# MoonLab-YH/AOD_MEH_HUA

Measured on AMD Instinct MI355X. Metric: images/sec train+HUA-score, RetinaNet-R50 VOC 512^2, higher is better.
Workload: dtype bf16x3

## Files before the change

aod_meh_hua_amd/_C.py:

```python
import ctypes as C
import os

import torch

_HERE = os.path.dirname(os.path.abspath(__file__))
LIB_PATH = os.environ.get('AOD_HIP_LIB') or os.path.join(_HERE, 'lib', 'libaodhip.so')


class AodHipError(RuntimeError):
    pass


if not os.path.exists(LIB_PATH):
    raise ImportError(f'{LIB_PATH} is missing: run `python -m aod_meh_hua_amd.build` (hipcc, gfx950). '
                      'There is no CPU fallback for the MEH/HUA hot path.')
lib = C.CDLL(LIB_PATH)


class ConvSeg(C.Structure):
    _fields_ = [('B', C.c_int32), ('H', C.c_int32), ('W', C.c_int32), ('OH', C.c_int32), ('OW', C.c_int32),
                ('src_row0', C.c_int64), ('dst_row0', C.c_int64)]


class ConvDesc(C.Structure):
    _fields_ = [('C', C.c_int32), ('N', C.c_int32), ('R', C.c_int32), ('S', C.c_int32), ('stride', C.c_int32),
                ('pad', C.c_int32), ('dil', C.c_int32), ('transposed', C.c_int32), ('relu', C.c_int32),
                ('out_f32', C.c_int32), ('nseg', C.c_int32), ('x3', C.c_int32), ('seg', ConvSeg * 8)]


P, I32, I64, F32, U64, SZ = C.c_void_p, C.c_int32, C.c_int64, C.c_float, C.c_uint64, C.c_size_t
_SIGS = {
    'aod_version': (C.c_int, []),
    'aod_conv_x3p_count': (C.c_int64, []),
    'aod_set_pointwise_mode': (C.c_int, [I32]),
    'aod_bottleneck64_fwd': (C.c_int, [P, I32, I32, I32, I32, P, P, P, P, P, P, P, P, P, P, P, P]),
    'aod_bottleneck64x3_fwd': (C.c_int, [P, I32, I32, I32, I32, P, P, P, P, P, P, P, P, P, P, P, P]),
    'aod_bottleneck64x3_ds_fwd': (C.c_int, [P, I32, I32, I32, P, P, P, P, P, P, P, P, P, P, P, P, P, P]),
    'aod_bottleneck64_ds_fwd': (C.c_int, [P, I32, I32, I32, P, P, P, P, P, P, P, P, P, P, P, P, P, P]),
    'aod_halo_conv3x3_x3_applies': (C.c_int, [P]),
    'aod_halo_conv3x3_x3': (C.c_int, [P, P, P, P, P, P]),
    'aod_mfma_clock_probe': (C.c_int, [I32, I32, P, P, P]),
    'aod_bottleneck128x3_bwd': (C.c_int, [P, I32, I32, I32, P, P, P, P, P, P, P, P, P, P, P, P, P]),
    'aod_bottleneck128x3_fwd': (C.c_int, [P, I32, I32, I32, P, P, P, P, P, P, P, P, P, P, P, P, P]),
    'aod_bottleneck128_fwd': (C.c_int, [P, I32, I32, I32, P, P, P, P, P, P, P, P, P, P, P, P, P]),
    'aod_frag_pack': (C.c_int, [P, I32, I32, P]),
    'aod_frag_pack_item_bytes': (C.c_int, []),
    'aod_bottleneck256f_fwd': (C.c_int, [P, I32, I32, I32, P, P, P, P, P, P, P, P, P, P, P, P, P]),
    'aod_bottleneck256f_bwd': (C.c_int, [P, I32, I32, I32, P, P, P, P, P, P, P, P, P, P, P, P, P]),
    'aod_bottleneck_bwd': (C.c_int, [I32, P, I32, I32, I32, P, P, P, P, P, P, P, P, P, P, P, P, P]),
    'aod_bottleneck256_fwd': (C.c_int, [P, I32, I32, I32, P, P, P, P, P, P, P, P, P, P, P, P, P]),
    'aod_conv2d': (C.c_int, [C.POINTER(ConvDesc), P, P, P, P, P, P, P, P, P, P, P]),
    'aod_conv2d_ws_bytes': (SZ, [C.POINTER(ConvDesc)]),
    'aod_conv2d_ws': (C.c_int, [C.POINTER(ConvDesc), P, P, P, P, P, P, P, P, P, P, P, SZ, P]),
    'aod_conv2d_grouped': (C.c_int, [C.POINTER(ConvDesc), I32, P, P, P, P, P, P, P]),
    'aod_halo_conv3x3_applies': (C.c_int, [C.POINTER(ConvDesc)]),
    'aod_halo_conv3x3': (C.c_int, [C.POINTER(ConvDesc), P, P, P, P, P, P, P]),
    'aod_conv2d_wgrad': (C.c_int, [C.POINTER(ConvDesc), P, P, P, P, P]),
    'aod_conv2d_wgrad_splits': (C.c_int, [C.POINTER(ConvDesc)]),
    'aod_conv2d_wgrad_slabs': (C.c_int, [C.POINTER(ConvDesc), P, P, P, I32, I64, P, P]),
    'aod_conv2d_wgrad_group_plan': (C.c_int, [P, I32, P]),
    'aod_conv2d_wgrad_grouped': (C.c_int, [P, I32, P, P, P, P, P, P, P]),
    'aod_unpack_wgrad_slabs_grouped': (C.c_int, [I32, P, P, P, P, P, P, P, P, P, P, P, P, P, P, P, P, P]),
    'aod_unpack_wgrad_slabs': (C.c_int, [P, I32, I64, P, I32, I32, I32, I32, I32, I32, P, P, P, P, P, P, P]),
    'aod_conv_row_table_bytes': (SZ, [C.POINTER(ConvDesc)]),
    'aod_conv_row_table': (C.c_int, [C.POINTER(ConvDesc), P, P]),
    'aod_pack_weight_fwd': (C.c_int, [P, P, I32, I32, I32, I32, I32, P]),
    'aod_param_prep': (C.c_int, [P, I32, I32, P]),
    'aod_param_prep_item_bytes': (C.c_int, []),
    'aod_pack_weight_dgrad': (C.c_int, [P, P, I32, I32, I32, I32, I32, P, P]),
    'aod_unpack_wgrad': (C.c_int, [P, P, I32, I32, I32, I32, I32, I32, I32, P, P, P, P, P, P, P]),
    'aod_nchw_f32_to_nhwc_bf16': (C.c_int, [P, P, I32, I32, I32, I32, I32, P]),
    'aod_nchw_f32_to_s2d_bf16': (C.c_int, [P, P, I32, I32, I32, I32, P]),
    'aod_stem_pool_fwd': (C.c_int, [P, P, P, P, P, I32, I32, I32, P]),
    'aod_set_deterministic': (C.c_int, [I32]),
    'aod_get_deterministic': (C.c_int, []),
    'aod_stem_pool_x3_fwd': (C.c_int, [P, P, P, P, P, I32, I32, I32, I32, P]),
    'aod_maxpool3x3s2': (C.c_int, [P, P, I32, I32, I32, I32, P]),
    'aod_upsample2x_add': (C.c_int, [P, P, I32, I32, I32, I32, I32, I32, P]),
    'aod_upsample2x_add_bwd': (C.c_int, [P, P, I32, I32, I32, I32, I32, I32, P]),
    'aod_upsample2x_add_to': (C.c_int, [P, P, P, I32, I32, I32, I32, I32, I32, P]),
    'aod_upsample2x_add_bwd_set': (C.c_int, [P, P, I32, I32, I32, I32, I32, I32, P]),
    'aod_act_bwd': (C.c_int, [P, P, P, P, P, P, P, P, P, P, I64, I32, I32, I32, P]),
    'aod_add_relu': (C.c_int, [P, P, P, I64, P]),
    'aod_pad_cast_colsum': (C.c_int, [P, P, P, P, I64, I32, I32, I32, P]),
    'aod_assign_ws_bytes': (SZ, [I32, I32]),
    'aod_max_iou_assign': (C.c_int, [P, P, I64, I32, P, P, P, I32, F32, F32, F32, I32, I32, P, P, P, P, P, P, P, P, P, I32, P, P]),
    'aod_loss_partials_len': (SZ, [I64]),
    'aod_edl_focal_l1_fwd': (C.c_int, [P, P, P, P, P, P, I64, I32, F32, F32, P, P, P, P]),
    'aod_edl_focal_l1_bwd': (C.c_int, [P, P, P, P, P, P, I64, I32, F32, F32, P, P, P, F32, I32, P, P, I32, I32, I32, I32, P]),
    'aod_edl_focal_elem': (C.c_int, [P, P, I64, I32, F32, F32, P, P, P]),
    'aod_meh_loss_fwd': (C.c_int, [P, P, P, I64, P, P, P]),
    'aod_meh_loss_bwd': (C.c_int, [P, P, P, I64, P, P, I32, I32, I32, P]),
    'aod_loss_levels_partials_len': (SZ, [I32, P]),
    'aod_edl_focal_l1_levels_fwd': (C.c_int, [P, P, P, P, P, P, I32, P, I32, F32, F32, P, P, P, P, I32, P, P, P]),
    'aod_edl_focal_l1_levels_bwd': (C.c_int, [P, P, P, P, P, P, I32, P, I32, F32, F32, P, P, P, P, P, I32, I32, I32, I32, P]),
    'aod_meh_loss_levels_fwd': (C.c_int, [P, P, P, I32, P, P, P, P]),
    'aod_meh_loss_levels_bwd': (C.c_int, [P, P, P, I32, P, P, P, I32, I32, I32, P]),
    'aod_softmax_rowmax': (C.c_int, [P, I32, I64, I32, F32, P, P, I32, P]),
    'aod_topk_stable': (C.c_int, [P, I32, I64, I32, P, I64, P]),
    'aod_pre_nms_levels': (C.c_int, [I32, P, P, P, P, P, P, I32, I32, F32, I32, I32, P, P, P, P, F32, P, P, P, P, P, P, P, I64, P]),
    'aod_gather_decode': (C.c_int, [P, P, P, P, P, I32, I64, I32, I32, I64, P, P, P, P, F32, P, P, P, P, I64, I64, I64, I32, P]),
    'aod_nms_ws_bytes': (SZ, [I32, I32, I32]),
    'aod_multiclass_nms': (C.c_int, [P, P, I32, I32, I32, F32, F32, I32, P, P, P, P, P, P]),
    'aod_hua_ws_bytes': (SZ, [I32, I32]),
    'aod_hua_score': (C.c_int, [P, P, P, P, P, P, P, P, P, I32, I32, I32, I32, I32, F32, F32, F32, I32, U64, P, I32, I32, I32, P, P, I32, P, P, P]),
    'aod_maxpool_fwd': (C.c_int, [P, P, I32, I32, I32, I32, I32, I32, I32, I32, I32, P]),
    'aod_maxpool_bwd': (C.c_int, [P, P, P, I32, I32, I32, I32, I32, I32, I32, I32, I32, P]),
    'aod_l2norm_fwd': (C.c_int, [P, P, P, I64, I32, F32, P]),
    'aod_l2norm_bwd': (C.c_int, [P, P, P, P, P, I64, I32, F32, P]),
    'aod_ssd_loss_fwd': (C.c_int, [P, P, P, P, P, P, I32, I32, I32, I32, I32, F32, P, P, P, P]),
    'aod_ssd_loss_bwd': (C.c_int, [P, P, P, P, P, P, P, P, I32, I32, I32, I32, F32, P, P, P, P, P, P]),
    'aod_synth_normal_images': (C.c_int, [P, I32, I64, U64, P, P]),
    'aod_image_xform': (C.c_int, [P, P, I32, I32, I32, P, P]),
    'aod_x3_split': (C.c_int, [P, P, I64, I32, P]),
    'aod_x3_merge': (C.c_int, [P, P, I64, I32, P]),
    'aod_x3_add': (C.c_int, [P, P, P, I64, P]),
    'aod_x3_nchw_f32_to_s2d': (C.c_int, [P, P, I32, I32, I32, I32, P]),
    'aod_x3_maxpool3x3s2': (C.c_int, [P, P, I32, I32, I32, I32, P]),
    'aod_x3_upsample2x_add_to': (C.c_int, [P, P, P, I32, I32, I32, I32, I32, I32, P]),
    'aod_x3_upsample2x_add_bwd_set': (C.c_int, [P, P, I32, I32, I32, I32, I32, I32, P]),
    'aod_x3_act_bwd': (C.c_int, [P, P, P, P, I64, I32, I32, P]),
    'aod_x3_pad_cast_colsum': (C.c_int, [P, P, P, P, I64, I32, P]),
    'aod_x3_nchw_f32_to_nhwc': (C.c_int, [P, P, I32, I32, I32, I32, P]),
    'aod_x3_maxpool_fwd': (C.c_int, [P, P, I32, I32, I32, I32, I32, I32, I32, I32, I32, P]),
    'aod_x3_maxpool_bwd': (C.c_int, [P, P, P, I32, I32, I32, I32, I32, I32, I32, I32, I32, P]),
    'aod_x3_l2norm_fwd': (C.c_int, [P, P, P, I64, I32, F32, P]),
    'aod_x3_l2norm_bwd': (C.c_int, [P, P, P, P, P, I64, I32, F32, P]),
    'aod_sgd_multi': (C.c_int, [P, P, P, P, I32, F32, P, F32, F32, I32, F32, P]),
}
for _n, (_r, _a) in _SIGS.items():
    if hasattr(lib, _n):
        getattr(lib, _n).restype = _r
        getattr(lib, _n).argtypes = _a
lib.aod_last_error.restype = C.c_char_p


def ptr(t):
    if t is None:
        return None
    if not t.is_cuda:
        raise AodHipError('aod_meh_hua_amd ops need tensors on the MI355X (cuda:N); got a CPU tensor. There is no CPU fallback.')
    return C.c_void_p(t.data_ptr())


def stream():
    return C.c_void_p(torch.cuda.current_stream().cuda_stream)


def check(rc, name='aod'):
    if rc != 0:
        raise AodHipError(f'{name} failed ({rc}): {lib.aod_last_error().decode()}')


def call(name, *args):
    check(getattr(lib, name)(*args), name)
```

aod_meh_hua_amd/csrc/conv.hip:

```cpp
#include "common.h"
#include "pointwise.h"
#include "conv_x3p.h"

struct ConvGroup { const bf16_t* x; const bf16_t* w; void* y; const float* pre_shift; const bf16_t* mask; float* colsum; };
struct ConvKParams {
  const bf16_t* x;
  const bf16_t* w;
  void* y;
  const float* pre_scale;
  const float* pre_shift;
  const bf16_t* res;
  const bf16_t* mask;
  const float* post_scale;
  bf16_t* zraw;
  float* colsum;
  int C, N, K, R, S, stride, pad, dil, transposed, relu, out_f32;
  int nseg, M;
  int tiles_m, tiles_n;
  int ksplit;
  float* ws;
  int perm;
  int ngroups;
  ConvGroup grp[4];
  int stagger;
// ... 879 lines not shown
    for (int j = 0; j < 8; ++j) sr[er][ec * 8 + j] = csum[j];
    __syncthreads();
    const int c = blockIdx.y * 256 + t;
    if (c < p.N) {
      float s2 = 0.f;
#pragma unroll
      for (int r = 0; r < 8; ++r) s2 += sr[r][t];
      if (p.cs_ws) p.cs_ws[(long long)blockIdx.x * p.N + c] = s2;
      else atomicAdd(p.colsum + c, s2);
    }
  }
}

static void x3p_args(const ConvKParams& p, X3PArgs& a) {
  memset(&a, 0, sizeof(a));
  a.x = p.x; a.w = p.w; a.y = reinterpret_cast<bf16_t*>(p.y); a.pre_scale = p.pre_scale; a.pre_shift = p.pre_shift; a.res = p.res; a.mask = p.mask;
  a.colsum = p.colsum; a.C = p.C; a.N = p.N; a.K = p.K; a.taps = p.R * p.S; a.S = p.S; a.stride = p.stride; a.pad = p.pad; a.dil = p.dil;
  a.transposed = p.transposed; a.relu = p.relu; a.nseg = p.nseg; a.M = p.M; a.x_bytes = p.x_bytes; a.w_bytes = p.w_bytes;
  a.tapin = (p.tap_inner && a.taps > 1 && p.C >= 256) ? 1 : 0;
  for (int i = 0; i < 8; ++i) {
    a.segH[i] = p.segH[i]; a.segW[i] = p.segW[i]; a.segOH[i] = p.segOH[i]; a.segOW[i] = p.segOW[i]; a.segB[i] = p.segB[i];
    a.seg_src0[i] = p.seg_src0[i]; a.seg_dst0[i] = p.seg_dst0[i]; a.seg_mend[i] = p.seg_mend[i];
  }
  if (p.ngroups > 1) {
    a.ngroups = p.ngroups;
    for (int g = 0; g < p.ngroups; ++g) {
      a.grp[g].x = p.grp[g].x; a.grp[g].w = p.grp[g].w; a.grp[g].y = reinterpret_cast<bf16_t*>(p.grp[g].y); a.grp[g].shift = p.grp[g].pre_shift;
      a.grp[g].mask = p.grp[g].mask; a.grp[g].colsum = p.grp[g].colsum;
    }
  }
}

static int choose_ksplit(const ConvKParams& p) {
  const int nk = (p.K + 63) / 64;
  if (nk < 64) return 1;
  static const char* dbg_hw = getenv("AOD_KSPLIT_MAXHW");
  const long long maxhw = dbg_hw ? atoll(dbg_hw) : 256;
  long long rows16 = 0;
  for (int i = 0; i < p.nseg; ++i) {
    if (p.segB[i] <= 0) continue;
    if ((long long)p.segOH[i] * p.segOW[i] > maxhw) return 1;
    rows16 += 16ll * p.segOH[i] * p.segOW[i];
  }
  static const char* dbg_ks = getenv("AOD_KSPLIT_STEPS");
  if (dbg_ks) { const int per = atoi(dbg_ks); return nk / per > 1 ? nk / per : 1; }
  const long long tiles = ((rows16 + 127) / 128) * ((p.N + 127) / 128);
  long long ks = 512 / (tiles > 0 ? tiles : 1);
  if (ks > nk / 8) ks = nk / 8;
  return ks > 1 ? (int)ks : 1;
}

static int conv_params(const aod_conv_desc_t* desc, const void* src, const void* w_packed, void* dst, const float* pre_scale,
                       const float* pre_shift, const void* res, const void* mask, const float* post_scale, void* zraw, float* colsum,
                       ConvKParams& p) {
  AOD_CHECK_ARG(desc && src && w_packed && dst, "conv: null pointer");
  memset(&p, 0, sizeof(p));
  int rc = fill_params(desc, p);
  if (rc) return rc;
  AOD_CHECK_ARG(!(desc->out_f32 && zraw), "conv: zraw needs a bf16 destination");
  if (desc->x3) {
    AOD_CHECK_ARG(!zraw && !post_scale, "conv (x3): zraw / post_scale are not supported");
    AOD_CHECK_ARG(desc->out_f32 || desc->N % 32 == 0, "conv (x3): a bf16 (X-layout) destination needs N %% 32 == 0, got %d", desc->N);
    AOD_CHECK_ARG(!(desc->out_f32 && (res || mask)), "conv (x3): residual / mask operands need an X-layout destination");
  }
  p.x = (const bf16_t*)src; p.w = (const bf16_t*)w_packed; p.y = dst;
  p.pre_scale = pre_scale; p.pre_shift = pre_shift; p.res = (const bf16_t*)res; p.mask = (const bf16_t*)mask;
  p.post_scale = post_scale; p.zraw = (bf16_t*)zraw; p.colsum = colsum;
  p.ksplit = 1;
  { static const char* dbg_st = getenv("AOD_STAGGER"); p.stagger = (dbg_st && dbg_st[0] == '0') ? 0 : 1; }
  { static const char* dbg_ti = getenv("AOD_X3_TAPS_INNER"); p.tap_inner = (dbg_ti && dbg_ti[0] == '0') ? 0 : 1; }
  p.perm = (desc->transposed && desc->stride == 2 && desc->R * desc->S > 1 && desc->R * desc->S <= 64) ? 1 : 0;
  if (desc->transposed && desc->stride == 2 && desc->R == 1 && desc->S == 1 && desc->pad == 0 && desc->nseg == 1 && res && res == dst &&
      !mask && !colsum && !pre_scale && !pre_shift && !post_scale && !zraw && !desc->relu && !desc->out_f32 && p.M > 0) {
    static const char* dbg_lat = getenv("AOD_DGRAD_LATTICE");
    if (!(dbg_lat && dbg_lat[0] == '0')) {
      p.up_w = p.segOW[0]; p.up_hw = p.segOH[0] * p.segOW[0];
      p.segOH[0] = p.segH[0]; p.segOW[0] = p.segW[0];
      p.stride = 1;
      const long long m = (long long)p.segB[0] * p.segH[0] * p.segW[0];
      p.M = (int)m;
      for (int i = 0; i < 8; ++i) p.seg_mend[i] = (int)m;
      p.bigrows = m >= (1ll << 22) ? 1 : 0;
    }
  }
  static const char* dbg_perm = getenv("AOD_DGRAD_CLASSES");
  if (dbg_perm && dbg_perm[0] == '0') p.perm = 0;
  long long xrows = 0;
  for (int i = 0; i < desc->nseg; ++i) {
    const aod_conv_seg_t& sg = desc->seg[i];
    AOD_CHECK_ARG(sg.src_row0 >= 0, "conv: negative src_row0");
    const long long e = sg.src_row0 + (long long)sg.B * sg.H * sg.W;
    if (e > xrows) xrows = e;
  }
  p.x_bytes = xrows * p.C * 2;
  p.w_bytes = (long long)p.N * p.K * 2;
  AOD_CHECK_ARG(p.x_bytes < 0xe0000000ll && p.w_bytes < 0xe0000000ll, "conv: operand larger than 3.5 GiB (32-bit buffer offsets)");
  return 0;
}

extern "C" size_t aod_conv2d_ws_bytes(const aod_conv_desc_t* desc) {
  ConvKParams p;
  memset(&p, 0, sizeof(p));
  if (!desc || fill_params(desc, p) != 0 || p.M == 0) return 0;
  const int ks = choose_ksplit(p);
  return ks > 1 ? (size_t)ks * p.M * p.N * 4 : 0;
}

extern "C" int aod_conv2d_ws(const aod_conv_desc_t* desc, const void* src, const void* w_packed, void* dst,
                             const float* pre_scale, const float* pre_shift, const void* res, const void* mask,
                             const float* post_scale, void* zraw, float* colsum, void* workspace, size_t workspace_bytes,
                             aod_stream_t stream) {
  ConvKParams p;
  int rc = conv_params(desc, src, w_packed, dst, pre_scale, pre_shift, res, mask, post_scale, zraw, colsum, p);
  if (rc) return rc;
  if (p.M == 0) return 0;
  hipStream_t st = (hipStream_t)stream;
  if (!p.x3 && !p.up_w && p.R == 1 && p.S == 1 && p.stride == 1 && p.pad == 0 && p.nseg == 1 && !p.out_f32 && !p.zraw && !p.post_scale) {
    PwArgs a;
    const long long s0 = p.seg_src0[0], d0 = p.seg_dst0[0];
    a.x = p.x + s0 * p.C; a.w = p.w; a.y = reinterpret_cast<bf16_t*>(p.y) + d0 * p.N;
    a.pre_scale = p.pre_scale; a.pre_shift = p.pre_shift;
    a.res = p.res ? p.res + d0 * p.N : nullptr; a.mask = p.mask ? p.mask + d0 * p.N : nullptr; a.colsum = p.colsum;
    a.M = p.M; a.N = p.N; a.K = p.C; a.relu = p.relu;
    if (aod_pw_wants(a)) return aod_pw_gemm(a, st);
  }
  const int ks = (workspace && !p.perm && !p.up_w) ? choose_ksplit(p) : 1;
  if (ks > 1) {
    const size_t need = (size_t)ks * p.M * p.N * 4;
    AOD_CHECK_ARG(workspace_bytes >= need, "conv: split-K workspace of %zu bytes, need %zu (aod_conv2d_ws_bytes)", workspace_bytes, need);
    p.ksplit = ks; p.ws = (float*)workspace;
    if (p.x3) { if (p.N > 64) launch_conv<128, 128, 256, 2, false, 2, true>(p, st); else launch_conv<128, 64, 256, 2, false, 2, true>(p, st); }
    else if (p.N > 64) launch_conv<128, 128>(p, st); else launch_conv<128, 64>(p, st);
    AOD_LAUNCH_CHECK();
    p.cs_ws = p.colsum ? aod_det_scratch((size_t)((p.M + 7) / 8) * p.N) : nullptr;
    hipLaunchKernelGGL(conv_splitk_finalize_kernel, dim3((p.M + 7) / 8, (p.N + 255) / 256), dim3(256), 0, st, p);
    AOD_LAUNCH_CHECK();
    if (p.cs_ws) return aod_colsum_finalize(p.cs_ws, (p.M + 7) / 8, p.N, p.N, p.colsum, nullptr, 0, st);
    return 0;
  }
  auto ntiles = [&](int bm, int bn) { return (long long)((p.M + bm - 1) / bm) * ((p.N + bn - 1) / bn); };
  static const char* dbg_want = getenv("AOD_TILE_WANT");
  const long long want = dbg_want ? atoll(dbg_want) : 512;
  const int pad128 = (p.N + 127) / 128 * 128, pad64 = (p.N + 63) / 64 * 64;
  const bool ragged = p.N > 128 && (pad128 - pad64) * 5 >= pad128;
  if (p.x3 && !p.out_f32 && !p.zraw && !p.post_scale && !p.bigrows && p.R == p.S) {
    const long long t256 = ntiles(256, 256);
    const bool big = !p.res && p.N % 256 == 0 && p.K >= 2048 && t256 >= 240 && t256 * 100 >= ((t256 + 255) / 256) * 256 * 92;
    const char* dbg_big = getenv("AOD_X3P_OVER_256");
    if (!big || (dbg_big && dbg_big[0] == '1')) {
      X3PArgs a;
      x3p_args(p, a);
      a.lat = p.perm ? 1 : (p.up_w ? 2 : 0);
      a.up_w = p.up_w; a.up_hw = p.up_hw;
      if (aod_conv_x3p_wants(a, p.colsum && aod_get_deterministic())) return aod_conv_x3p_launch(a, st);
    }
  }
  if (p.x3) {
    {
      static const char* dbg_t256x = getenv("AOD_TILE_256");
      const long long t256 = ntiles(256, 256);
      const bool fits = t256 >= 240 && t256 * 100 >= ((t256 + 255) / 256) * 256 * 92;
      if (!(dbg_t256x && dbg_t256x[0] == '0') && !p.res && !p.out_f32 && p.N % 256 == 0 && p.K >= 2048 && fits) {
        if (!p.mask) launch_conv<256, 256, 512, 0, false, 2, true>(p, st); else launch_conv<256, 256, 512, 1, false, 2, true>(p, st);
        AOD_LAUNCH_CHECK();
        return 0;
      }
    }
    {
      const char* dbg_t192 = getenv("AOD_X3_TILE_192");
      const long long t192 = ntiles(192, 192);
      if (!(dbg_t192 && dbg_t192[0] == '0') && p.N > 128 && p.N <= 192 && !p.res && !p.mask && !p.zraw && p.K >= 2048 && t192 >= 240) {
        launch_conv<192, 192, 512, 0, false, 2, true>(p, st);
        AOD_LAUNCH_CHECK();
        return 0;
      }
    }
    static const char* dbg_w8x = getenv("AOD_X3_128_W8");
    const long long t128 = ntiles(128, 128);
    const bool w8 = dbg_w8x && dbg_w8x[0] == '1' && !p.res && !p.out_f32 && p.N % 128 == 0 && t128 >= 256;
    if (w8) {
      if (!p.mask) launch_conv<128, 128, 512, 0, false, 2, true>(p, st); else launch_conv<128, 128, 512, 1, false, 2, true>(p, st);
      AOD_LAUNCH_CHECK();
      return 0;
    }
    static const char* dbg_st3 = getenv("AOD_X3_128_ST3");
    if (ragged && ntiles(128, 64) >= want) launch_conv<128, 64, 256, 2, false, 2, true>(p, st);
    else if (p.N > 64 && dbg_st3 && dbg_st3[0] == '1' && ntiles(128, 128) >= 256) launch_conv<128, 128, 256, 2, false, 3, true>(p, st);
    else if (p.N > 64 && ntiles(128, 128) >= want) launch_conv<128, 128, 256, 2, false, 2, true>(p, st);
    else if (p.N > 64 && ntiles(64, 128) >= want) launch_conv<64, 128, 256, 2, false, 3, true>(p, st);
    else if (p.N <= 64 && ntiles(128, 64) >= want) launch_conv<128, 64, 256, 2, false, 2, true>(p, st);
    else if (p.N > 64 && ntiles(128, 64) >= want && p.N % 128 != 0) launch_conv<128, 64, 256, 2, false, 2, true>(p, st);
    else launch_conv<64, 64, 256, 2, false, 3, true>(p, st);
    AOD_LAUNCH_CHECK();
    return 0;
  }
  static const char* dbg_t256 = getenv("AOD_TILE_256");
  const long long t256 = ntiles(256, 256);
  const bool fits256 = t256 >= 240 && t256 * 100 >= ((t256 + 255) / 256) * 256 * 92;
  if (!(dbg_t256 && dbg_t256[0] == '0') && !p.res && !p.out_f32 && p.N % 256 == 0 && p.K >= 1024 &&
      ((dbg_t256 && dbg_t256[0] == '1' && t256 >= 128) || fits256)) {
    if (!p.mask) launch_conv<256, 256, 512, 0>(p, st); else launch_conv<256, 256, 512, 1>(p, st);
    AOD_LAUNCH_CHECK();
    return 0;
  }
  static const char* dbg_w8 = getenv("AOD_TILE_W8");
  if (!(dbg_w8 && dbg_w8[0] == '0') && !p.res && p.N >= 128 && p.K >= 1024 && ntiles(128, 128) >= want) {
    if (!p.mask) launch_conv<128, 128, 512, 0>(p, st); else launch_conv<128, 128, 512, 1>(p, st);
    AOD_LAUNCH_CHECK();
    return 0;
  }
  static const char* dbg_r3 = getenv("AOD_RING3");
  const bool r3 = !(dbg_r3 && dbg_r3[0] == '0') && p.K >= 256;
  if (ragged && ntiles(128, 64) >= want) launch_conv<128, 64>(p, st);
  else if (p.N > 64 && ntiles(128, 128) >= want) launch_conv<128, 128>(p, st);
  else if (p.N > 64 && ntiles(64, 128) >= want) { if (r3) launch_conv<64, 128, 256, 2, false, 3>(p, st); else launch_conv<64, 128>(p, st); }
  else if (p.N <= 64 && ntiles(128, 64) >= want) launch_conv<128, 64>(p, st);
  else if (p.N > 64 && ntiles(128, 64) >= want && p.N % 128 != 0) launch_conv<128, 64>(p, st);
  else { if (r3) launch_conv<64, 64, 256, 2, false, 3>(p, st); else launch_conv<64, 64>(p, st); }
  AOD_LAUNCH_CHECK();
  return 0;
}

extern "C" int aod_conv2d_grouped(const aod_conv_desc_t* desc, int ngroups, const void* const* src, const void* const* w_packed,
                                  void* const* dst, const float* const* pre_shift, const void* const* mask, float* const* colsum,
                                  aod_stream_t stream) {
  AOD_CHECK_ARG(desc && src && w_packed && dst && ngroups >= 1 && ngroups <= 4, "conv_grouped: 1..4 groups");
  AOD_CHECK_ARG(!desc->out_f32, "conv_grouped: bf16 destinations only");
  AOD_CHECK_ARG(!desc->x3 || (desc->N % 256 == 0 && desc->R * desc->S * desc->C >= 2048), "conv_grouped (x3): N %% 256 == 0 and a deep K required");
  ConvKParams p;
  int rc = conv_params(desc, src[0], w_packed[0], dst[0], nullptr, pre_shift ? pre_shift[0] : nullptr, nullptr, mask ? mask[0] : nullptr, nullptr,
                       nullptr, colsum ? colsum[0] : nullptr, p);
  if (rc) return rc;
  if (p.M == 0) return 0;
  AOD_CHECK_ARG(!p.perm, "conv_grouped: class-major stride-2 dgrad launches are not grouped");
  p.ngroups = ngroups;
  bool any_mask = false;
  for (int g = 0; g < ngroups; ++g) {
    AOD_CHECK_ARG(src[g] && w_packed[g] && dst[g], "conv_grouped: null operand in group %d", g);
    p.grp[g].x = (const bf16_t*)src[g]; p.grp[g].w = (const bf16_t*)w_packed[g]; p.grp[g].y = dst[g];
    p.grp[g].pre_shift = pre_shift ? pre_shift[g] : nullptr;
    p.grp[g].mask = mask ? (const bf16_t*)mask[g] : nullptr;
    p.grp[g].colsum = colsum ? colsum[g] : nullptr;
    any_mask = any_mask || p.grp[g].mask;
  }
  hipStream_t st = (hipStream_t)stream;
  auto fill = [&](int bm, int bn, int slots) {
    const long long t = (long long)((p.M + bm - 1) / bm) * ((p.N + bn - 1) / bn) * ngroups;
    return (double)t / (double)(((t + slots - 1) / slots) * slots);
  };
  static const char* dbg_t256 = getenv("AOD_TILE_256");
  const bool ok256 = !(dbg_t256 && dbg_t256[0] == '0') && p.N % 256 == 0 && p.K >= 1024;
  if (p.x3 && p.R == p.S && !p.bigrows) {
    const char* dbg_g = getenv("AOD_X3P_GROUPED");
    bool any_cs = false;
    for (int g = 0; g < ngroups; ++g) any_cs = any_cs || p.grp[g].colsum;
    if (dbg_g && dbg_g[0] == '1') {
      X3PArgs a;
      x3p_args(p, a);
      if (ngroups == 1) { a.ngroups = 1; a.grp[0].x = p.grp[0].x; a.grp[0].w = p.grp[0].w; a.grp[0].y = reinterpret_cast<bf16_t*>(p.grp[0].y);
                          a.grp[0].shift = p.grp[0].pre_shift; a.grp[0].mask = p.grp[0].mask; a.grp[0].colsum = p.grp[0].colsum; }
      if (aod_conv_x3p_wants(a, any_cs && aod_get_deterministic())) return aod_conv_x3p_launch(a, st);
    }
  }
  if (p.x3) {
    if (!any_mask) launch_conv<256, 256, 512, 0, true, 2, true>(p, st); else launch_conv<256, 256, 512, 1, true, 2, true>(p, st);
  } else if (ok256 && fill(256, 256, 256) * 1.12 >= fill(128, 128, 512)) {
    if (!any_mask) launch_conv<256, 256, 512, 0, true>(p, st); else launch_conv<256, 256, 512, 1, true>(p, st);
  } else {
    AOD_CHECK_ARG(p.N >= 128, "conv_grouped: N >= 128 required");
    if (!any_mask) launch_conv<128, 128, 512, 0, true>(p, st); else launch_conv<128, 128, 512, 1, true>(p, st);
  }
  AOD_LAUNCH_CHECK();
  return 0;
}

extern "C" int aod_conv2d(const aod_conv_desc_t* desc, const void* src, const void* w_packed, void* dst,
                          const float* pre_scale, const float* pre_shift, const void* res, const void* mask,
                          const float* post_scale, void* zraw, float* colsum, aod_stream_t stream) {
  return aod_conv2d_ws(desc, src, w_packed, dst, pre_scale, pre_shift, res, mask, post_scale, zraw, colsum, nullptr, 0, stream);
}

struct RowRec {
  unsigned xrow;
  unsigned zoff;
  unsigned wc2;
  unsigned pad_;
  unsigned long long mask;
  unsigned long long pad2_;
};
static_assert(sizeof(RowRec) == 32, "row record layout");

__global__ void row_table_kernel(const ConvKParams p, RowRec* __restrict__ tab) {
  const int m = blockIdx.x * 256 + threadIdx.x;
  if (m >= p.M) return;
  int sg = 0, mstart = 0;
  while (sg < p.nseg - 1 && m >= p.seg_mend[sg]) { mstart = p.seg_mend[sg]; ++sg; }
  const int ml = m - mstart;
  const int ohw = p.segOH[sg] * p.segOW[sg];
  const int b = ml / ohw, rem = ml - b * ohw;
  const int oy = rem / p.segOW[sg], ox = rem - oy * p.segOW[sg];
  const int H = p.segH[sg], W = p.segW[sg];
  const int y0 = oy * p.stride - p.pad, x0 = ox * p.stride - p.pad;
  RowRec r;
  r.xrow = (unsigned)((p.seg_src0[sg] + (long long)b * H * W + (long long)y0 * W + x0) * p.C * 2);
  r.zoff = (unsigned)((p.seg_dst0[sg] + ml) * (long long)p.N * 2);
  r.wc2 = (unsigned)(W * p.C * 2);
// ... 1013 lines not shown
```

aod_meh_hua_amd/csrc/conv_x3p.h:

```cpp
#pragma once
#include "common.h"

struct X3PArgs {
  const bf16_t* x;
  const bf16_t* w;
  bf16_t* y;
  const float* pre_scale;
  const float* pre_shift;
  const bf16_t* res;
  const bf16_t* mask;
  float* colsum;
  int C, N, K, taps, S, stride, pad, dil, transposed, relu, tapin;
  int nseg, M, tiles_m, tiles_n;
  int rot;
  int lat;
  int up_w, up_hw;
  int ngroups;
  struct { const bf16_t* x; const bf16_t* w; bf16_t* y; const float* shift; const bf16_t* mask; float* colsum; } grp[4];
  long long x_bytes, w_bytes;
  int segH[8], segW[8], segOH[8], segOW[8], segB[8];
  long long seg_src0[8], seg_dst0[8];
  int seg_mend[8];
};

int aod_conv_x3p_wants(const X3PArgs& a, int deterministic_colsum);
int aod_conv_x3p_launch(const X3PArgs& a, hipStream_t st);
```

include/aod_hip.h:

```cpp
#ifndef AOD_HIP_H
#define AOD_HIP_H
#include <stddef.h>
#include <stdint.h>

#ifdef __cplusplus
extern "C" {
#endif

typedef void* aod_stream_t;

const char* aod_last_error(void);
int aod_version(void);

typedef struct {
  int32_t B, H, W;
  int32_t OH, OW;
  int64_t src_row0;
  int64_t dst_row0;
} aod_conv_seg_t;

typedef struct {
  int32_t C, N;
  int32_t R, S;
  int32_t stride, pad, dil;
  int32_t transposed;
  int32_t relu;
  int32_t out_f32;
  int32_t nseg;
  int32_t x3;
  aod_conv_seg_t seg[8];
} aod_conv_desc_t;

int aod_conv2d(const aod_conv_desc_t* desc, const void* src, const void* w_packed, void* dst,
               const float* pre_scale, const float* pre_shift, const void* res, const void* mask,
               const float* post_scale, void* zraw, float* colsum, aod_stream_t stream);

size_t aod_conv2d_ws_bytes(const aod_conv_desc_t* desc);
int aod_conv2d_ws(const aod_conv_desc_t* desc, const void* src, const void* w_packed, void* dst,
                  const float* pre_scale, const float* pre_shift, const void* res, const void* mask,
                  const float* post_scale, void* zraw, float* colsum, void* workspace, size_t workspace_bytes,
                  aod_stream_t stream);

int64_t aod_conv_x3p_count(void);

int aod_set_pointwise_mode(int mode);

int aod_set_deterministic(int on);
int aod_get_deterministic(void);

int aod_bottleneck64_fwd(const void* x, int Cin, int B, int H, int W, const void* w1, const float* s1, const float* b1, const void* w2,
                         const float* s2, const float* b2, const void* w3, const float* s3, const float* b3, const void* res, void* y,
                         aod_stream_t stream);
int aod_bottleneck64_ds_fwd(const void* x, int B, int H, int W, const void* w1, const float* s1, const float* b1, const void* w2,
                            const float* s2, const float* b2, const void* w3, const float* s3, const float* b3, const void* wd,
                            const float* sd, const float* bd, void* y, aod_stream_t stream);
int aod_bottleneck128_fwd(const void* x, int B, int H, int W, const void* w1, const float* s1, const float* b1, const void* w2,
                          const float* s2, const float* b2, const void* w3, const float* s3, const float* b3, void* y, void* t1, void* t2,
                          aod_stream_t stream);
int aod_bottleneck256_fwd(const void* x, int B, int H, int W, const void* w1, const float* s1, const float* b1, const void* w2,
                          const float* s2, const float* b2, const void* w3, const float* s3, const float* b3, void* y, void* t1, void* t2,
                          aod_stream_t stream);
int aod_bottleneck_bwd(int planes, const void* g, int B, int H, int W, const void* wd3, const void* wd2, const void* wd1, const void* act_t2,
                       const void* act_t1, const void* act_x, void* gx, void* gt2, void* gt1, float* colsum_t2, float* colsum_t1,
                       float* colsum_x, aod_stream_t stream);

int aod_frag_pack_item_bytes(void);
int aod_frag_pack(const void* items_dev, int nitems, int total_blocks, aod_stream_t stream);
int aod_bottleneck256f_fwd(const void* x, int B, int H, int W, const void* w1f, const float* s1, const float* b1, const void* w2f,
                           const float* s2, const float* b2, const void* w3f, const float* s3, const float* b3, void* y, void* t1, void* t2,
                           aod_stream_t stream);
int aod_bottleneck256f_bwd(const void* g, int B, int H, int W, const void* wd3f, const void* wd2f, const void* wd1f, const void* act_t2,
                           const void* act_t1, const void* act_x, void* gx, void* gt2, void* gt1, float* colsum_t2, float* colsum_t1,
                           float* colsum_x, aod_stream_t stream);

int aod_conv2d_grouped(const aod_conv_desc_t* desc, int ngroups, const void* const* src, const void* const* w_packed, void* const* dst,
                       const float* const* pre_shift, const void* const* mask, float* const* colsum, aod_stream_t stream);

int aod_conv2d_wgrad(const aod_conv_desc_t* desc, const void* x, const void* dz, float* dw_f32,
                     const void* row_table, aod_stream_t stream);
int aod_conv2d_wgrad_splits(const aod_conv_desc_t* desc);
int aod_conv2d_wgrad_slabs(const aod_conv_desc_t* desc, const void* x, const void* dz, float* slabs, int nslabs, int64_t slab_stride,
                           const void* row_table, aod_stream_t stream);
int aod_conv2d_wgrad_group_plan(const aod_conv_desc_t* const* descs, int n, int32_t* splits_out);
int aod_conv2d_wgrad_grouped(const aod_conv_desc_t* const* descs, int n, const void* const* x, const void* const* dz, float* const* slabs,
                             const int32_t* nslabs, const int64_t* slab_stride, const void* const* row_table, aod_stream_t stream);
size_t aod_conv_row_table_bytes(const aod_conv_desc_t* desc);
int aod_conv_row_table(const aod_conv_desc_t* desc, void* table, aod_stream_t stream);

int aod_pack_weight_fwd(const float* w_oihw, void* w_packed, int O, int I, int R, int S, int Ipad, aod_stream_t stream);
int aod_pack_weight_dgrad(const float* w_oihw, void* w_packed, int O, int I, int R, int S, int Opad, const float* scale,
                          aod_stream_t stream);
int aod_unpack_wgrad(float* dw_orsi, float* grad_oihw, int O, int I, int R, int S, int Ipad, int accumulate, int clear_src,
                     const float* scale, const float* w_oihw, float* wdot, const float* bn_s1, const float* bn_mean,
                     const float* bn_invstd, aod_stream_t stream);

int aod_unpack_wgrad_slabs(const float* dw_slabs, int nslabs, int64_t slab_stride, float* grad_oihw, int O, int I, int R, int S, int Ipad,
                           int accumulate, const float* scale, const float* w_oihw, float* wdot, const float* bn_s1,
                           const float* bn_mean, const float* bn_invstd, aod_stream_t stream);

int aod_unpack_wgrad_slabs_grouped(int n, const float* const* dw_slabs, const int32_t* nslabs, const int64_t* slab_stride, float* const* g,
                                   const int32_t* O, const int32_t* I, const int32_t* R, const int32_t* S, const int32_t* Ipad,
                                   const int32_t* accumulate, const float* const* scale, const float* const* w_oihw, float* const* wdot,
                                   const float* const* bn_s1, const float* const* bn_mean, const float* const* bn_invstd,
                                   aod_stream_t stream);
int aod_param_prep(const void* items_dev, int nitems, int total_blocks, aod_stream_t stream);
int aod_param_prep_item_bytes(void);

int aod_nchw_f32_to_nhwc_bf16(const float* src, void* dst, int B, int C, int H, int W, int Cpad, aod_stream_t stream);
int aod_nchw_f32_to_s2d_bf16(const float* src, void* dst, int B, int C, int H, int W, aod_stream_t stream);
int aod_stem_pool_fwd(const void* x_s2d, const void* w_packed, const float* scale, const float* shift, void* y, int B, int H2, int W2,
                      aod_stream_t stream);
int aod_maxpool3x3s2(const void* src, void* dst, int B, int H, int W, int C, aod_stream_t stream);
int aod_upsample2x_add(const void* src, void* dst, int B, int h, int w, int C, int H, int W, aod_stream_t stream);
int aod_upsample2x_add_bwd(const void* g_dst, void* g_src_accum, int B, int h, int w, int C, int H, int W, aod_stream_t stream);
int aod_upsample2x_add_to(const void* top, const void* lateral, void* out, int B, int h, int w, int C, int H, int W, aod_stream_t stream);
int aod_upsample2x_add_bwd_set(const void* g_dst, void* g_src, int B, int h, int w, int C, int H, int W, aod_stream_t stream);
int aod_act_bwd(const void* g, const void* a, const void* z, const float* scale, const float* mean, const float* invstd,
                void* dz, void* gmask_out, float* dbeta, float* dgamma, int64_t M, int N, int relu, int g_is_f32,
                aod_stream_t stream);
int aod_pad_cast_colsum(const void* g, const float* relu_out_f32, void* dz, float* colsum, int64_t M, int N, int Npad,
                        int g_is_f32, aod_stream_t stream);
int aod_add_relu(const void* a, const void* b, void* out, int64_t n, aod_stream_t stream);

int aod_halo_conv3x3_applies(const aod_conv_desc_t* desc);
int aod_halo_conv3x3(const aod_conv_desc_t* desc, const void* src, const void* w_packed, void* dst, const float* pre_shift,
                     const void* mask, float* colsum, aod_stream_t stream);

size_t aod_loss_partials_len(int64_t nrows);
int aod_edl_focal_l1_fwd(const float* cls, const int64_t* labels, const float* label_w,
                         const float* bbox_pred, const float* bbox_tgt, const float* bbox_w,
                         int64_t nrows, int C, float gamma, float alpha,
                         float* loss_noR, float* sums3, float* partials, aod_stream_t stream);
int aod_edl_focal_l1_bwd(const float* cls, const int64_t* labels, const float* label_w,
                         const float* bbox_pred, const float* bbox_tgt, const float* bbox_w,
                         int64_t nrows, int C, float gamma, float alpha,
                         const float* g_cls, const float* g_bbox, const float* g_noR, float g_noR_scalar, int g_noR_is_scalar,
                         void* grad_cls, void* grad_bbox, int out_bf16, int A, int pitch_cls, int pitch_box,
                         aod_stream_t stream);
int aod_edl_focal_elem(const float* cls, const int64_t* labels, int64_t nrows, int C, float gamma, float alpha,
                       const float* grad_out, float* out, aod_stream_t stream);
int aod_meh_loss_fwd(const float* lam, const float* loss_noR, const float* bbox_w4, int64_t n,
                     float* out_sum, float* partials, aod_stream_t stream);
int aod_meh_loss_bwd(const float* lam, const float* loss_noR, const float* bbox_w4, int64_t n,
                     const float* g, void* grad_lam, int out_bf16, int A, int pitch, aod_stream_t stream);
size_t aod_loss_levels_partials_len(int nlevels, const int64_t* level_rows);
int aod_edl_focal_l1_levels_fwd(const float* cls, const int64_t* labels, const float* label_w,
                                const float* bbox_pred, const float* bbox_tgt, const float* bbox_w,
                                int nlevels, const int64_t* level_rows, int C, float gamma, float alpha,
                                float* loss_noR, float* sums, float* partials, const int32_t* num_pos, int num_images,
                                float* divisors, float* num_total, aod_stream_t stream);
int aod_edl_focal_l1_levels_bwd(const float* cls, const int64_t* labels, const float* label_w,
                                const float* bbox_pred, const float* bbox_tgt, const float* bbox_w,
                                int nlevels, const int64_t* level_rows, int C, float gamma, float alpha,
                                const float* g_sums, const float* divisors, const float* g_noR_rows, void* grad_cls, void* grad_bbox, int out_bf16,
                                int A, int pitch_cls, int pitch_box, aod_stream_t stream);
int aod_meh_loss_levels_fwd(const float* lam, const float* loss_noR, const float* bbox_w4, int nlevels, const int64_t* level_rows,
                            float* out_sums, float* partials, aod_stream_t stream);
int aod_meh_loss_levels_bwd(const float* lam, const float* loss_noR, const float* bbox_w4, int nlevels, const int64_t* level_rows,
                            const float* g, void* grad_lam, int out_bf16, int A, int pitch, aod_stream_t stream);

size_t aod_assign_ws_bytes(int B, int Gmax);
int aod_max_iou_assign(const float* anchors, const uint8_t* valid, int64_t A, int B,
                       const float* gts, const int32_t* gt_count, const int64_t* gt_labels, int Gmax,
                       float pos_thr, float neg_thr, float min_pos_iou, int gt_max_assign_all, int num_classes,
                       const float* means4, const float* stds4,
                       int64_t* assigned, int64_t* labels, float* label_w, float* bbox_t, float* bbox_w,
                       int32_t* num_pos, void* ws, int nlev, const int64_t* level_start_host, aod_stream_t stream);

int aod_softmax_rowmax(const float* cls, int B, int64_t rows_per_img, int C, float fg_thr, float* rowmax, int32_t* any_fg,
                       int has_bg, aod_stream_t stream);
int aod_topk_stable(const float* score, int B, int64_t A, int k, int32_t* idx, int64_t out_pitch, aod_stream_t stream);
int aod_gather_decode(const float* cls, const float* reg, const float* lam_map, const float* anchors, const int32_t* idx,
                      int B, int64_t A, int k, int C, int64_t idx_pitch, const float* img_hw, const float* scale4,
                      const float* means4, const float* stds4, float wh_ratio_clip, float* boxes, float* scores, float* lam,
                      int32_t* cand_anchor, int64_t n_total, int64_t cand0, int64_t anchor0, int normalize, aod_stream_t stream);
int aod_pre_nms_levels(int L, const float* const* cls, const float* const* reg, const float* const* lam_map, const float* const* anchors,
                       const int64_t* A, const int32_t* k, int B, int C, float fg_thr, int has_bg, int normalize, const float* img_hw,
                       const float* scale4, const float* means4, const float* stds4, float wh_ratio_clip, float* rowmax, int32_t* any_fg,
                       int32_t* idx, float* boxes, float* scores, float* lam, int32_t* cand_anchor, int64_t n_total, aod_stream_t stream);
size_t aod_nms_ws_bytes(int B, int n, int C);
int aod_multiclass_nms(const float* boxes, const float* scores, int B, int n, int C, float score_thr, float iou_thr,
                       int max_num, float* dets, int64_t* det_labels, int64_t* keep, int32_t* num_det,
                       void* ws, aod_stream_t stream);

size_t aod_hua_ws_bytes(int B, int max_pairs);
int aod_hua_score(const float* boxes, const float* scores, const float* lam, const int32_t* cand_anchor,
                  const float* dets, const int32_t* num_det, const int32_t* level_start_host, const int32_t* level_any_fg,
                  const int64_t* image_ids, int B, int n, int L, int C, int max_num, float obj_score_thr, float obj_iou_thr,
                  float fg_thr, int num_samples, uint64_t seed, const int32_t* agg3_host, int clsW, int scale_mode,
                  int dirichlet_cols, float* unc, float* pair_out, int max_pairs, int32_t* pair_count, void* ws, aod_stream_t stream);

int aod_maxpool_fwd(const void* x, void* y, int B, int H, int W, int C, int OH, int OW, int k, int s, int p, aod_stream_t stream);
int aod_maxpool_bwd(const void* x, const void* g, void* gx, int B, int H, int W, int C, int OH, int OW, int k, int s, int p,
                    aod_stream_t stream);
int aod_l2norm_fwd(const void* x, const float* w, void* y, int64_t rows, int C, float eps, aod_stream_t stream);
int aod_l2norm_bwd(const void* x, const float* w, const void* g, void* gx, float* gw, int64_t rows, int C, float eps, aod_stream_t stream);
// ... 73 lines not shown
```

Measured before the change: 651.3.

## Add warp-specialized persistent 1x1 conv kernel with resident activation tile

Adds a new persistent kernel for 1x1 stride-1 x3 (split-bf16) convolutions, routed ahead of the existing x3p path. Producer waves stream weight tiles into a 3-slot LDS ring using buffer-to-LDS loads. The full 64-row activation strip stays resident in LDS across all output-channel tiles, and consumer waves run MFMA with fused scale, shift, residual, mask, relu and colsum epilogues. The aim is to reuse activations across N tiles and overlap weight loads with compute. The cost is a large LDS footprint, only 2 waves per EU, and atomic colsum accumulation.

```diff
diff --git a/aod_meh_hua_amd/_C.py b/aod_meh_hua_amd/_C.py
--- a/aod_meh_hua_amd/_C.py
+++ b/aod_meh_hua_amd/_C.py
@@ -32,6 +32,8 @@
 _SIGS = {
     'aod_version': (C.c_int, []),
     'aod_conv_x3p_count': (C.c_int64, []),
+    'aod_conv_x3r_count': (C.c_int64, []),
+    'aod_set_x3r_mode': (C.c_int, [I32]),
     'aod_set_pointwise_mode': (C.c_int, [I32]),
     'aod_bottleneck64_fwd': (C.c_int, [P, I32, I32, I32, I32, P, P, P, P, P, P, P, P, P, P, P, P]),
     'aod_bottleneck64x3_fwd': (C.c_int, [P, I32, I32, I32, I32, P, P, P, P, P, P, P, P, P, P, P, P]),
diff --git a/aod_meh_hua_amd/csrc/conv.hip b/aod_meh_hua_amd/csrc/conv.hip
--- a/aod_meh_hua_amd/csrc/conv.hip
+++ b/aod_meh_hua_amd/csrc/conv.hip
@@ -1055,6 +1055,7 @@
       x3p_args(p, a);
       a.lat = p.perm ? 1 : (p.up_w ? 2 : 0);
       a.up_w = p.up_w; a.up_hw = p.up_hw;
+      if (aod_conv_x3r_wants(a, p.colsum && aod_get_deterministic())) return aod_conv_x3r_launch(a, st);
       if (aod_conv_x3p_wants(a, p.colsum && aod_get_deterministic())) return aod_conv_x3p_launch(a, st);
     }
   }
diff --git a/aod_meh_hua_amd/csrc/conv_x3p.h b/aod_meh_hua_amd/csrc/conv_x3p.h
--- a/aod_meh_hua_amd/csrc/conv_x3p.h
+++ b/aod_meh_hua_amd/csrc/conv_x3p.h
@@ -25,3 +25,6 @@
 
 int aod_conv_x3p_wants(const X3PArgs& a, int deterministic_colsum);
 int aod_conv_x3p_launch(const X3PArgs& a, hipStream_t st);
+
+int aod_conv_x3r_wants(const X3PArgs& a, int deterministic_colsum);
+int aod_conv_x3r_launch(const X3PArgs& a, hipStream_t st);
diff --git a/aod_meh_hua_amd/csrc/conv_x3r.hip b/aod_meh_hua_amd/csrc/conv_x3r.hip
--- /dev/null
+++ b/aod_meh_hua_amd/csrc/conv_x3r.hip
@@ -0,0 +1,319 @@
+#include "conv_x3p.h"
+
+#include <stdlib.h>
+
+namespace {
+
+constexpr int XR_TM = 64, XR_BN = 256;
+constexpr int XR_XCHUNK = XR_TM * 128;
+constexpr int XR_STAGE = XR_BN * 128;
+constexpr int XR_NL = 8;
+constexpr int XR_MAXCC = 8;
+constexpr unsigned XR_OOB = 0xf0000000u;
+constexpr int XR_SLOTS = 3;
+static_assert(XR_SLOTS * XR_STAGE + XR_MAXCC * XR_XCHUNK <= 160 * 1024, "LDS");
+
+template <int PRE, int XR_RING>
+__global__ __launch_bounds__(512) __attribute__((amdgpu_waves_per_eu(2, 2))) void conv_x3r_kernel(const X3PArgs p) {
+  constexpr int XR_FLY = XR_RING - 2, XR_XBASE = XR_RING * XR_STAGE;
+  extern __shared__ __attribute__((aligned(16))) char smem[];
+  const int lane = threadIdx.x & 63;
+  const int wave = __builtin_amdgcn_readfirstlane((int)(threadIdx.x >> 6));
+  const int G = (int)gridDim.x, bid = (int)blockIdx.x;
+  const int nitems = p.tiles_m;
+  const int nmine = (nitems - bid + G - 1) / G;
+  const int CC = p.C >> 6;
+  const int NCT = p.tiles_n;
+  const int T = NCT * CC;
+
+  if (wave >= 4) {
+    const int w = wave - 4;
+    const int prow = lane >> 3;
+    const int kc = (lane & 7) ^ ((4 * w + (lane >> 4)) & 7);
+    unsigned wvo[XR_NL];
+#pragma unroll
+    for (int i = 0; i < XR_NL; ++i) {
+      const int R = 8 * w + 32 * i + prow;
+      const int wv = R >> 6, nb = (R >> 4) & 3;
+      const int nrel = wv * 64 + (nb >> 1) * 32 + ((R >> 2) & 3) * 8 + (nb & 1) * 4 + (R & 3);
+      wvo[i] = (unsigned)((nrel * p.K + kc * 8) * 2);
+    }
+    const auto rsrc_x = __builtin_amdgcn_make_buffer_rsrc((void*)p.x, 0, (int)p.x_bytes, 0x00020000);
+    const auto rsrc_w = __builtin_amdgcn_make_buffer_rsrc((void*)p.w, 0, (int)p.w_bytes, 0x00020000);
+    const unsigned rowb = (unsigned)(p.C * 2);
+    char* const lds_w = smem + (8 * w) * 128;
+    char* const lds_x = smem + XR_XBASE + (8 * w) * 128;
+    for (int j = 0; j < nmine; ++j) {
+      const int m0 = (bid + j * G) * XR_TM;
+      unsigned vo[2];
+#pragma unroll
+      for (int i = 0; i < 2; ++i) {
+        const int m = m0 + 8 * w + 32 * i + prow;
+        vo[i] = m < p.M ? (unsigned)(p.seg_src0[0] + m) * rowb + (unsigned)(kc * 16) : XR_OOB;
+      }
+      for (int cc = 0; cc < CC; ++cc) {
+#pragma unroll
+        for (int i = 0; i < 2; ++i)
+          __builtin_amdgcn_raw_ptr_buffer_load_lds(rsrc_x, (__attribute__((address_space(3))) void*)(lds_x + cc * XR_XCHUNK + i * 4096), 16, vo[i],
+                                                   (unsigned)cc * 128u, 0, 0);
+      }
+      int issued = 0, slot = 0;
+      for (int ct = 0; ct < NCT; ++ct) {
+        const unsigned soff_w0 = (unsigned)(ct * XR_BN) * (unsigned)(p.K * 2);
+        for (int cc = 0; cc < CC; ++cc) {
+          char* const sa = lds_w + slot * XR_STAGE;
+          const unsigned soff_w = soff_w0 + (unsigned)cc * 128u;
+#pragma unroll
+          for (int i = 0; i < XR_NL; ++i)
+            __builtin_amdgcn_raw_ptr_buffer_load_lds(rsrc_w, (__attribute__((address_space(3))) void*)(sa + i * 4096), 16, wvo[i], soff_w, 0, 0);
+          ++issued;
+          slot = slot == XR_RING - 1 ? 0 : slot + 1;
+          if (issued > XR_FLY) {
+            asm volatile("s_waitcnt vmcnt(%0)" ::"n"(XR_NL * XR_FLY) : "memory");
+            __builtin_amdgcn_s_barrier();
+          }
+        }
+      }
+      asm volatile("s_waitcnt vmcnt(0)" ::: "memory");
+      for (int k = (T > XR_FLY ? T - XR_FLY : 0); k < T + 1; ++k) __builtin_amdgcn_s_barrier();
+    }
+    return;
+  }
+
+  const int wn = wave;
+  const int lr = lane & 15, lq = lane >> 4;
+  const int sw = (lr >> 1) & 7;
+  const int oh = (lq ^ sw) << 4, ol = ((4 + lq) ^ sw) << 4;
+  const int xoff = XR_XBASE + lr * 128, woff = (wn * 64 + lr) * 128;
+  const int NP = ((p.N + 31) >> 5) << 6;
+  typedef __attribute__((ext_vector_type(4))) unsigned u32x4_t;
+  const auto rsrc_s = __builtin_amdgcn_make_buffer_rsrc((void*)p.pre_scale, 0, p.pre_scale ? p.N * 4 : 0, 0x00020000);
+  const auto rsrc_b = __builtin_amdgcn_make_buffer_rsrc((void*)p.pre_shift, 0, p.pre_shift ? p.N * 4 : 0, 0x00020000);
+  bf16_t* const gy = p.y;
+  const bf16_t* const gmask = p.mask;
+  float* const gcs = p.colsum;
+
+  for (int j = 0; j < nmine; ++j) {
+    const int m0 = (bid + j * G) * XR_TM;
+    bool live[4];
+    long long prow_[4];
+#pragma unroll
+    for (int mb = 0; mb < 4; ++mb) {
+      const int m = m0 + mb * 16 + lr;
+      live[mb] = m < p.M;
+      const int mc = live[mb] ? m : p.M - 1;
+      prow_[mb] = (p.seg_dst0[0] + mc) * NP;
+    }
+    __builtin_amdgcn_s_barrier();
+    int cslot = 0;
+    for (int ct = 0; ct < NCT; ++ct) {
+      const int n0 = ct * XR_BN;
+      f32x4 acc[4][4];
+#pragma unroll
+      for (int nb = 0; nb < 4; ++nb)
+#pragma unroll
+        for (int mb = 0; mb < 4; ++mb) acc[nb][mb] = (f32x4){0.f, 0.f, 0.f, 0.f};
+      bf16x8 prh[PRE ? 2 : 1][4], prl[PRE == 1 ? 2 : 1][4];
+      if constexpr (PRE != 0) {
+        const bf16_t* const src = PRE == 1 ? p.res : gmask;
+#pragma unroll
+        for (int aa = 0; aa < 2; ++aa) {
+          const int col = 2 * (n0 + wn * 64 + 32 * aa) + 8 * lq;
+#pragma unroll
+          for (int mb = 0; mb < 4; ++mb) {
+            prh[aa][mb] = *reinterpret_cast<const bf16x8*>(src + prow_[mb] + col);
+            if constexpr (PRE == 1) prl[aa][mb] = *reinterpret_cast<const bf16x8*>(src + prow_[mb] + col + 32);
+          }
+        }
+        __builtin_amdgcn_sched_barrier(0);
+      }
+      for (int ks = 0; ks < CC; ++ks) {
+        const char* const st = smem + cslot * XR_STAGE;
+        const char* const xs = smem + ks * XR_XCHUNK;
+        cslot = cslot == XR_RING - 1 ? 0 : cslot + 1;
+        bf16x8 xh[4], xl[4], wh[4], wl[4];
+#pragma unroll
+        for (int q = 0; q < 4; ++q) xh[q] = *reinterpret_cast<const bf16x8*>(xs + xoff + oh + q * 2048);
+#pragma unroll
+        for (int q = 0; q < 4; ++q) wh[q] = *reinterpret_cast<const bf16x8*>(st + woff + oh + q * 2048);
+#pragma unroll
+        for (int q = 0; q < 4; ++q)
+#pragma unroll
+          for (int mb = 0; mb < 4; ++mb) acc[q][mb] = __builtin_amdgcn_mfma_f32_16x16x32_bf16(wh[q], xh[mb], acc[q][mb], 0, 0, 0);
+#pragma unroll
+        for (int q = 0; q < 4; ++q) xl[q] = *reinterpret_cast<const bf16x8*>(xs + xoff + ol + q * 2048);
+#pragma unroll
+        for (int q = 0; q < 4; ++q)
+#pragma unroll
+          for (int mb = 0; mb < 4; ++mb) acc[q][mb] = __builtin_amdgcn_mfma_f32_16x16x32_bf16(wh[q], xl[mb], acc[q][mb], 0, 0, 0);
+#pragma unroll
+        for (int q = 0; q < 4; ++q) wl[q] = *reinterpret_cast<const bf16x8*>(st + woff + ol + q * 2048);
+#pragma unroll
+        for (int q = 0; q < 4; ++q)
+#pragma unroll
+          for (int mb = 0; mb < 4; ++mb) acc[q][mb] = __builtin_amdgcn_mfma_f32_16x16x32_bf16(wl[q], xh[mb], acc[q][mb], 0, 0, 0);
+        asm volatile("s_waitcnt lgkmcnt(0)" ::: "memory");
+        __builtin_amdgcn_s_barrier();
+      }
+
+      float cs1[2][8], cb1[2][8], csum[2][8];
+      bf16x8 rh[2][4], rl[2][4], mh[2][4];
+#pragma unroll
+      for (int aa = 0; aa < 2; ++aa) {
+        const int cb = n0 + wn * 64 + 32 * aa + 8 * lq;
+        const int col = 2 * (cb - 8 * lq) + 8 * lq;
+        const u32x4_t b0 = __builtin_amdgcn_raw_buffer_load_b128(rsrc_b, cb * 4, 0, 0), b1 = __builtin_amdgcn_raw_buffer_load_b128(rsrc_b, cb * 4 + 16, 0, 0);
+        u32x4_t s0 = {0u, 0u, 0u, 0u}, s1 = {0u, 0u, 0u, 0u};
+        if (p.pre_scale) { s0 = __builtin_amdgcn_raw_buffer_load_b128(rsrc_s, cb * 4, 0, 0); s1 = __builtin_amdgcn_raw_buffer_load_b128(rsrc_s, cb * 4 + 16, 0, 0); }
+#pragma unroll
+        for (int q = 0; q < 4; ++q) {
+          cb1[aa][q] = __uint_as_float(b0[q]); cb1[aa][4 + q] = __uint_as_float(b1[q]);
+          cs1[aa][q] = __uint_as_float(s0[q]); cs1[aa][4 + q] = __uint_as_float(s1[q]);
+        }
+#pragma unroll
+        for (int mb = 0; mb < 4; ++mb) {
+          if constexpr (PRE == 1) { rh[aa][mb] = prh[aa][mb]; rl[aa][mb] = prl[aa][mb]; }
+          else if (p.res) {
+            rh[aa][mb] = *reinterpret_cast<const bf16x8*>(p.res + prow_[mb] + col);
+            rl[aa][mb] = *reinterpret_cast<const bf16x8*>(p.res + prow_[mb] + col + 32);
+          }
+          if constexpr (PRE == 2) mh[aa][mb] = prh[aa][mb];
+          else if (gmask) mh[aa][mb] = *reinterpret_cast<const bf16x8*>(gmask + prow_[mb] + col);
+        }
+      }
+#pragma unroll
+      for (int aa = 0; aa < 2; ++aa) {
+        const int col = 2 * (n0 + wn * 64 + 32 * aa) + 8 * lq;
+#pragma unroll
+        for (int q = 0; q < 8; ++q) csum[aa][q] = 0.f;
+#pragma unroll
+        for (int mb = 0; mb < 4; ++mb) {
+          float v[8];
+#pragma unroll
+          for (int q = 0; q < 4; ++q) { v[q] = acc[2 * aa][mb][q]; v[4 + q] = acc[2 * aa + 1][mb][q]; }
+          if (p.pre_scale) {
+#pragma unroll
+            for (int q = 0; q < 8; ++q) v[q] *= cs1[aa][q];
+          }
+#pragma unroll
+          for (int q = 0; q < 8; ++q) v[q] += cb1[aa][q];
+          if (p.res) {
+#pragma unroll
+            for (int q = 0; q < 8; ++q) v[q] += (float)rh[aa][mb][q] + (float)rl[aa][mb][q];
+          }
+          if (gmask) {
+#pragma unroll
+            for (int q = 0; q < 8; ++q) v[q] = ((float)mh[aa][mb][q] > 0.f) ? v[q] : 0.f;
+          }
+          if (p.relu) {
+#pragma unroll
+            for (int q = 0; q < 8; ++q) v[q] = fmaxf(v[q], 0.f);
+          }
+          bf16x8 ov, ovl;
+#pragma unroll
+          for (int q = 0; q < 8; ++q) { csum[aa][q] += live[mb] ? v[q] : 0.f; ov[q] = (bf16_t)v[q]; }
+#pragma unroll
+          for (int q = 0; q < 8; ++q) ovl[q] = (bf16_t)(v[q] - (float)ov[q]);
+          if (live[mb]) {
+            *reinterpret_cast<bf16x8*>(gy + prow_[mb] + col) = ov;
+            *reinterpret_cast<bf16x8*>(gy + prow_[mb] + col + 32) = ovl;
+          }
+        }
+      }
+      if (gcs) {
+        float mine = 0.f;
+#pragma unroll
+        for (int aa = 0; aa < 2; ++aa)
+#pragma unroll
+          for (int q = 0; q < 8; ++q) {
+            float s = csum[aa][q];
+            s += __shfl_xor(s, 1, 64); s += __shfl_xor(s, 2, 64); s += __shfl_xor(s, 4, 64); s += __shfl_xor(s, 8, 64);
+            mine = lr == aa * 8 + q ? s : mine;
+          }
+        atomicAdd(gcs + n0 + wn * 64 + 32 * (lr >> 3) + 8 * lq + (lr & 7), mine);
+      }
+    }
+  }
+}
+
+long long g_x3r_count = 0;
+int g_x3r_mode = -1;
+
+int xr_env_mode() {
+  static const int m = [] {
+    const char* e = getenv("AOD_X3R");
+    return !e ? 1 : (e[0] == '0' ? 0 : (e[0] == '2' ? 2 : 1));
+  }();
+  return m;
+}
+
+int xr_mode() {
+  const int m = __atomic_load_n(&g_x3r_mode, __ATOMIC_RELAXED);
+  return m >= 0 ? m : xr_env_mode();
+}
+
+int xr_cus() {
+  static int cus[64];
+  int dev = 0;
+  if (hipGetDevice(&dev) != hipSuccess || dev < 0 || dev > 63) dev = 0;
+  int n = __atomic_load_n(&cus[dev], __ATOMIC_RELAXED);
+  if (!n) {
+    if (hipDeviceGetAttribute(&n, hipDeviceAttributeMultiprocessorCount, dev) != hipSuccess || n <= 0) n = 256;
+    __atomic_store_n(&cus[dev], n, __ATOMIC_RELAXED);
+  }
+  return n;
+}
+
+template <int PRE, int RING>
+void xr_launch(const X3PArgs& a, int grid, hipStream_t st) {
+  const size_t lds = (size_t)RING * XR_STAGE + (size_t)(a.C >> 6) * XR_XCHUNK;
+  static unsigned long long attr = 0;
+  if (aod_first_on_device(&attr))
+    (void)hipFuncSetAttribute(reinterpret_cast<const void*>(&conv_x3r_kernel<PRE, RING>), hipFuncAttributeMaxDynamicSharedMemorySize, 160 * 1024);
+  hipLaunchKernelGGL((conv_x3r_kernel<PRE, RING>), dim3(grid), dim3(512), lds, st, a);
+}
+
+}
+
+static bool xr_routed(const X3PArgs& a) {
+  const long long items = ((long long)a.M + XR_TM - 1) / XR_TM;
+  return items >= 2ll * xr_cus();
+}
+
+int aod_conv_x3r_wants(const X3PArgs& a, int deterministic_colsum) {
+  const int mode = xr_mode();
+  if (mode == 0) return 0;
+  if (a.taps != 1 || a.stride != 1 || a.pad != 0 || a.lat != 0 || a.ngroups > 1 || a.nseg != 1) return 0;
+  if (a.segH[0] != a.segOH[0] || a.segW[0] != a.segOW[0]) return 0;
+  if (a.C % 64 != 0 || a.C < 128 || a.C > 64 * XR_MAXCC || a.K != a.C) return 0;
+  if (a.N % XR_BN != 0 || a.N < 512 || a.M <= 0) return 0;
+  if (deterministic_colsum) return 0;
+  if ((long long)a.K * 2 * a.N >= 0x7fffffffll) return 0;
+  if (a.M >= (1 << 22) || a.seg_dst0[0] + a.M >= (1ll << 31) || (a.seg_src0[0] + a.M) * (long long)a.C * 2 >= 0xe0000000ll) return 0;
+  if (mode != 2 && !xr_routed(a)) return 0;
+  if (a.transposed) {
+    const char* dg = getenv("AOD_X3P_DGRAD");
+    if (dg && dg[0] == '0') return 0;
+  }
+  return 1;
+}
+
+int aod_conv_x3r_launch(const X3PArgs& a0, hipStream_t st) {
+  X3PArgs a = a0;
+  a.tiles_m = (a.M + XR_TM - 1) / XR_TM;
+  a.tiles_n = a.N / XR_BN;
+  const int ncu = xr_cus();
+  const int grid = a.tiles_m < ncu ? a.tiles_m : ncu;
+  if (a.res) xr_launch<1, XR_SLOTS>(a, grid, st);
+  else if (a.mask) xr_launch<2, XR_SLOTS>(a, grid, st);
+  else xr_launch<0, XR_SLOTS>(a, grid, st);
+  AOD_LAUNCH_CHECK();
+  __atomic_add_fetch(&g_x3r_count, 1, __ATOMIC_RELAXED);
+  return 0;
+}
+
+extern "C" int64_t aod_conv_x3r_count(void) { return (int64_t)__atomic_load_n(&g_x3r_count, __ATOMIC_RELAXED); }
+
+extern "C" int aod_set_x3r_mode(int mode) {
+  return __atomic_exchange_n(&g_x3r_mode, mode < -1 || mode > 2 ? -1 : mode, __ATOMIC_RELAXED);
+}
diff --git a/include/aod_hip.h b/include/aod_hip.h
--- a/include/aod_hip.h
+++ b/include/aod_hip.h
@@ -42,6 +42,9 @@
                   aod_stream_t stream);
 
 int64_t aod_conv_x3p_count(void);
+
+int64_t aod_conv_x3r_count(void);
+int aod_set_x3r_mode(int mode);
 
 int aod_set_pointwise_mode(int mode);
 
```

Measured after the change: 650.6, median of 2. No clear change (-0.1%).
